# lucidrains/phenaki-pytorch

Measured on AMD Instinct MI355X. Metric: cvivit_encode_frames_per_sec, higher is better.
Workload: dtype bf16; 1 GPU; BASELINE configs[1]: C-ViViT (dim 512, patch 32, tpatch 2, depth 4+4, LFQ 65536) encode video -> token ids, (8,3,17,256,256) f32 per GPU resident in HBM; global_batch=8, parallelism=batch-shard x1, no data-path collective, hip_graph=True

## Files before the change

### include/phenaki_hip.h

```cpp
#ifndef PHENAKI_HIP_H
#define PHENAKI_HIP_H

#ifdef __cplusplus
extern "C" {
#endif

#define PK_OK 0
#define PK_EINVAL (-1)
#define PK_EALIGN (-2)
#define PK_ELAUNCH (-3)

int pk_gemm(int dtype, int a_is_f32, const void* A, int lda, const void* W, int ldw, int M, int N, int K,
            const float* bias, const float* res, int ldr, void* C, int ldc, int out_is_f32, int act,
            const int* a_rows, void* stream);

int pk_gemm_ex(int dtype, int a_is_f32, const void* A, int lda, const void* W, int ldw, int M, int N, int K,
               const float* bias, const float* res, int ldr, void* C, int ldc, int out_is_f32, int act,
               const int* a_rows, int a_nrows, int variant, void* C2, int ldc2, const float* ln_s, const float* ln_t,
               float ln_eps, const int* row_off, const int* col_off, float* stats_out, const float* ln_stats, int dup_rows,
               void* stream);
int pk_gemm_auto_variant(int dtype, int a_is_f32, int M, int N, int K, int lda, int ldw, int a_nrows);

int pk_layernorm(const float* x, int ldx, const float* gamma, const float* beta, float eps, void* out, int ldo,
                 int out_kind, float* out2, int ldo2, void* raw, int ldraw, int M, int D, int grp, int gstride,
// ... 220 lines not shown
                          const float* gscale_dev, void* stream);
int pk_ema_multi(const long long* table, int count, float weight, void* stream);
int pk_attn_train_prep(const float* q, long long ldq, const float* kv, long long ldkv, const float* null_kv, const float* q_scale, const float* k_scale,
                       float scale, float* Qh, float* Kh, float* Vh, int S, int heads, int n, int n_kv, int nnull, void* stream);
int pk_attn_train_prep_bwd(const float* q, long long ldq, const float* kv, long long ldkv, const float* null_kv, const float* q_scale, const float* k_scale,
                           float scale, const float* dQh, const float* dKh, const float* dVh, float* dq, long long lddq, float* dkv, long long lddkv,
                           float* pq, float* pk, float* dnull, int S, int heads, int n, int n_kv, int nnull, void* stream);
int pk_attn_bwd_work(int S, int heads, int n, int n_kv, int nnull);
int pk_attn_bwd_ws(const float* Qh, const float* Kh, const float* Vh, const void* O, long long ldo, int o_bf16, const float* dO, long long lddo,
                   const float* bias, const unsigned char* kmask, const float* slopes, int causal, float* dQh, float* dKh, float* dVh, float* dS,
                   float* lse, float* Drow, int S, int heads, int n, int n_kv, int nnull, int split_bf16, float* work, long long work_floats,
                   const pk_dropout* drop, void* stream);

int pk_im2col(const float* x, int B, int H, int W, int C, int kh, int kw, int stride, int pad, float* cols, long long ldc, void* stream);
int pk_col2im(const float* cols, long long ldc, int B, int H, int W, int C, int kh, int kw, int stride, int pad, float* dx, void* stream);
int pk_nchw_to_rows(const float* img, int B, int C, int H, int W, int Cp, float* rows, void* stream);
int pk_rows_to_nchw(const float* rows, int B, int C, int H, int W, int Cp, float* img, void* stream);
int pk_pick_frames(float* video, const int* frame, int B, int C, int F, int H, int W, float* img, int place, void* stream);
int pk_bmm(const float* A, long long lda, long long sA, int tA, const float* B, long long ldb, long long sB, int tB, float* C, long long ldc,
           long long sC, int batch, int M, int N, int K, int accumulate, void* stream);
int pk_row_softmax(const float* a, const float* b, const float* c, float* out, long long M, int n, int mode, void* stream);
int pk_row_l2scale(const float* x, const float* sc, const float* dz, const float* gx, const float* gsc, float* o0, float* o1, float* o2,
                   long long M, int d, int mode, void* stream);
int pk_row_ln_bwd2(const float* x, const float* gamma, const float* dy, const float* u, const float* w, float eps, float* grad_x,
                   float* grad_gamma_rows, float* grad_dy, long long M, int D, void* stream);

int pk_conv3x3(int dtype, int a_is_f32, const void* x, int B, int H, int W, int C, const void* Wm, int ldw, int Co, const float* bias, int act,
               const void* gate, int ldg, int gate_is_f32, void* y, int ldy, int out_is_f32, int tile, void* stream);
int pk_maxpool2x2(int is_f32, const void* x, int B, int H, int W, int C, void* y, void* stream);
int pk_maxpool2x2_bwd(int is_f32, const void* x, const float* dy, int B, int H, int W, int C, float* dx, void* stream);
int pk_adaptive_avgpool(int is_f32, const void* x, int B, int H, int W, int C, float* out, void* stream);
int pk_adaptive_avgpool_bwd(const float* dy, int B, int H, int W, int C, float* dx, void* stream);

int pk_frame_sqerr_parts(int H, int W);
int pk_frame_ssim_parts(int H, int W);
int pk_frame_sqerr(const float* a, const float* b, int B, int C, int F, int H, int W, float clamp_hi, float data_range, double* partials,
                   long long nparts, float* mse, float* psnr, void* stream);
int pk_frame_ssim(const float* a, const float* b, int B, int C, int F, int H, int W, float clamp_hi, float data_range, double* partials,
                  long long nparts, float* ssim, void* stream);
int pk_code_usage(const int* counts, int V, double* out, void* stream);

int pk_set_cache_policy(unsigned mask);
int pk_get_cache_policy();

int pk_gemm_epilogue_form(int dtype, int variant, int ln_kind, int vec_ok, int act, int out_is_f32, int has_bias, int has_res, int has_c2,
                          int has_stats_out, int has_scatter, int dup_rows, int pol, int pol_res);
int pk_gemm_ex_form(int dtype, int a_is_f32, const void* A, int lda, const void* W, int ldw, int M, int N, int K, const float* bias,
                    const float* res, int ldr, void* C, int ldc, int out_is_f32, int act, const int* a_rows, int a_nrows, int variant,
                    void* C2, int ldc2, const float* ln_s, const float* ln_t, float ln_eps, const int* row_off, const int* col_off,
                    float* stats_out, const float* ln_stats, int dup_rows);
int pk_set_gemm_hot_forms(int on);
int pk_get_gemm_hot_forms();

#ifdef __cplusplus
}
#endif
#endif
```

### phenaki_pytorch_amd/_lib.py

```python
import ctypes
import os

import torch

_HERE = os.path.dirname(os.path.abspath(__file__))
LIB_PATH = os.environ.get('PK_LIB_PATH') or os.path.join(_HERE, 'libphenaki_hip.so')

_P = ctypes.c_void_p
_I = ctypes.c_int
_F = ctypes.c_float
_L = ctypes.c_long
_LL = ctypes.c_longlong
_ULL = ctypes.c_ulonglong

SIGNATURES = {
    'pk_gemm': [_I, _I, _P, _I, _P, _I, _I, _I, _I, _P, _P, _I, _P, _I, _I, _I, _P, _P],
    'pk_gemm_ex': [_I, _I, _P, _I, _P, _I, _I, _I, _I, _P, _P, _I, _P, _I, _I, _I, _P, _I, _I, _P, _I, _P, _P, _F, _P, _P, _P, _P, _I, _P],
    'pk_gemm_auto_variant': [_I, _I, _I, _I, _I, _I, _I, _I],
    'pk_layernorm': [_P, _I, _P, _P, _F, _P, _I, _I, _P, _I, _P, _I, _I, _I, _I, _I, _I, _I, _I, _P],
    'pk_rmsnorm': [_P, _I, _P, _F, _P, _P, _I, _I, _I, _I, _P],
    'pk_gated_gelu_tanh': [_P, _I, _P, _I, _I, _I, _I, _P],
    'pk_l2norm_rows': [_P, _I, _P, _I, _I, _I, _I, _P],
    'pk_patchify_ln': [_P, _I, _I, _I, _I, _I, _I, _I, _I, _I, _I, _P, _P, _F, _P, _I, _I, _P],
    'pk_patch_embed': [_P, _I, _I, _I, _I, _I, _I, _I, _I, _F, _I,
# ... 76 lines not shown
    'pk_mul': [_P, _P, _P, _LL, _P],
    'pk_peg_wgrad_parts': [_LL],
    'pk_peg_bwd': [_P, _P, _P, _P, _P, _I, _I, _I, _I, _I, _I, _P],
    'pk_embed_bwd': [_P, _P, _F, _P, _P, _I, _I, _I, _P],
    'pk_bias_gather': [_P, _I, _P, _I, _P, _I, _I, _P],
    'pk_bias_scatter': [_P, _P, _I, _P, _I, _I, _I, _P],
    'pk_sum_batch': [_P, _LL, _I, _P, _LL, _P],
    'pk_sum_batch_multi': [_P, _I, _P],
    'pk_peg_adjoint': [_P, _P, _P, _I, _I, _I, _I, _I, _I, _P],
    'pk_colsum_multi': [_P, _I, _P],
    'pk_reduce_multi': [_P, _I, _P, _I, _P],
    'pk_pack_multi': [_P, _I, _P],
    'pk_pack_table_prepare': [_P, _I],
    'pk_pack_table': [_P, _I, _I, _P],
    'pk_bce_head': [_P, _LL, _P, _P, _P, _F, _P, _P, _P, _P, _LL, _P, _P, _I, _I, _P],
    'pk_attn_train_prep': [_P, _LL, _P, _LL, _P, _P, _P, _F, _P, _P, _P, _I, _I, _I, _I, _I, _P],
    'pk_attn_train_prep_bwd': [_P, _LL, _P, _LL, _P, _P, _P, _F, _P, _P, _P, _P, _LL, _P, _LL, _P, _P, _P, _I, _I, _I, _I, _I, _P],
    'pk_gemm_splitk': [_I, _P, _I, _P, _I, _I, _I, _I, _I, _P, _I, _P, _I, _P],
    'pk_adamw': [_P, _P, _P, _P, _F, _F, _F, _F, _F, _I, _LL, _P],
    'pk_adamw_multi': [_P, _I, _F, _F, _F, _F, _F, _I, _P],
    'pk_grad_sumsq_parts': [_P, _I],
    'pk_grad_sumsq': [_P, _I, _P, _LL, _P],
    'pk_grad_clip_coef': [_P, _LL, _F, _P, _P],
    'pk_scale_multi': [_P, _I, _P, _P],
    'pk_adamw_multi_scaled': [_P, _I, _F, _F, _F, _F, _F, _I, _P, _P],
    'pk_ema_multi': [_P, _I, _F, _P],
    'pk_attn_bwd_ws': [_P, _P, _P, _P, _LL, _I, _P, _LL, _P, _P, _P, _I, _P, _P, _P, _P, _P, _P, _I, _I, _I, _I, _I, _I, _P, _LL, _P, _P],
    'pk_attn_bwd_work': [_I, _I, _I, _I, _I],
    'pk_im2col': [_P, _I, _I, _I, _I, _I, _I, _I, _I, _P, _LL, _P],
    'pk_col2im': [_P, _LL, _I, _I, _I, _I, _I, _I, _I, _I, _P, _P],
    'pk_nchw_to_rows': [_P, _I, _I, _I, _I, _I, _P, _P],
    'pk_rows_to_nchw': [_P, _I, _I, _I, _I, _I, _P, _P],
    'pk_pick_frames': [_P, _P, _I, _I, _I, _I, _I, _P, _I, _P],
    'pk_bmm': [_P, _LL, _LL, _I, _P, _LL, _LL, _I, _P, _LL, _LL, _I, _I, _I, _I, _I, _P],
    'pk_row_softmax': [_P, _P, _P, _P, _LL, _I, _I, _P],
    'pk_row_l2scale': [_P, _P, _P, _P, _P, _P, _P, _P, _LL, _I, _I, _P],
    'pk_row_ln_bwd2': [_P, _P, _P, _P, _P, _F, _P, _P, _P, _LL, _I, _P],
    'pk_conv3x3': [_I, _I, _P, _I, _I, _I, _I, _P, _I, _I, _P, _I, _P, _I, _I, _P, _I, _I, _I, _P],
    'pk_maxpool2x2': [_I, _P, _I, _I, _I, _I, _P, _P],
    'pk_maxpool2x2_bwd': [_I, _P, _P, _I, _I, _I, _I, _P, _P],
    'pk_adaptive_avgpool': [_I, _P, _I, _I, _I, _I, _P, _P],
    'pk_adaptive_avgpool_bwd': [_P, _I, _I, _I, _I, _P, _P],
    'pk_frame_sqerr_parts': [_I, _I],
    'pk_frame_ssim_parts': [_I, _I],
    'pk_frame_sqerr': [_P, _P, _I, _I, _I, _I, _I, _F, _F, _P, _LL, _P, _P, _P],
    'pk_frame_ssim': [_P, _P, _I, _I, _I, _I, _I, _F, _F, _P, _LL, _P, _P],
    'pk_code_usage': [_P, _I, _P, _P],
    'pk_set_cache_policy': [ctypes.c_uint],
    'pk_get_cache_policy': [],
    'pk_gemm_epilogue_form': [_I] * 14,
    'pk_gemm_ex_form': [_I, _I, _P, _I, _P, _I, _I, _I, _I, _P, _P, _I, _P, _I, _I, _I, _P, _I, _I, _P, _I, _P, _P, _F, _P, _P, _P, _P, _I],
    'pk_set_gemm_hot_forms': [_I],
    'pk_get_gemm_hot_forms': [],
}

_ERR = {-1: 'PK_EINVAL (bad shape/size/flag)', -2: 'PK_EALIGN (pointer/stride alignment)', -3: 'PK_ELAUNCH (HIP launch failed)'}

_lib = None
_AB_OPTIONAL = ('pk_set_cache_policy', 'pk_get_cache_policy', 'pk_gemm_epilogue_form', 'pk_gemm_ex_form', 'pk_set_gemm_hot_forms', 'pk_get_gemm_hot_forms',
                'pk_vocab_ce_reg', 'pk_ce_grad_slab_reg', 'pk_vocab_weight_mean', 'pk_vocab_weight_mean_words')


def load():
    global _lib
    if _lib is None:
        if not os.path.exists(LIB_PATH):
            raise RuntimeError(f'{LIB_PATH} is missing: run `python -m phenaki_pytorch_amd.build` '
                               '(the MI355X build has no CPU / eager fallback)')
        lib = ctypes.CDLL(LIB_PATH)
        for name, args in SIGNATURES.items():
            if name in _AB_OPTIONAL and 'PK_LIB_PATH' in os.environ and not hasattr(lib, name):
                continue
            fn = getattr(lib, name)
            fn.argtypes = args
            fn.restype = _I
        _lib = lib
    return _lib


def _check(rc, name):
    if rc != 0:
        raise RuntimeError(f'{name} failed: {_ERR.get(rc, rc)}')


def ptr(t):
    return None if t is None else t.data_ptr()


def f32p(t, name='parameter', rows_ok=False):
    if t is None:
        return None
    if t.dtype != torch.float32 or not (t.is_contiguous() or (rows_ok and t.stride(-1) == 1)):
        raise RuntimeError(f'{name}: the MI355X kernels read this tensor as contiguous float32, got {t.dtype} '
                           f'{"contiguous" if t.is_contiguous() else "strided"} (keep the module in float32; the compute '
                           'precision is chosen with set_compute_dtype, not with .half()/.bfloat16())')
    return t.data_ptr()


def stream(t=None):
    if t is None:
        return torch.cuda.current_stream().cuda_stream
    idx = t.device.index
    cur = _current_device()
    if idx is not None and idx != cur:
        raise RuntimeError(f'operand on cuda:{idx} but the current device is cuda:{cur}: '
                           'call torch.cuda.set_device(...) first (one process per GPU)')
    return _raw_stream(cur)


_raw_stream = getattr(torch._C, '_cuda_getCurrentRawStream', None) or (lambda i: torch.cuda.current_stream(i).cuda_stream)
_current_device = getattr(torch._C, '_cuda_getDevice', None) or torch.cuda.current_device


def require_device(t, name='tensor'):
    if not t.is_cuda:
        raise RuntimeError(f'{name} is on {t.device}: the MI355X build runs on HIP devices only (no CPU fallback)')


F32, BF16, BF16X3 = 0, 1, 2
ACT_NONE, ACT_GEGLU, ACT_LEAKY, ACT_RELU = 0, 1, 2, 3


def tdtype(dtype):
    return torch.bfloat16 if dtype == BF16 else torch.float32


def split_planes(w32):
    n, k = w32.shape
    assert k % 32 == 0 and w32.dtype == torch.float32
    hi = w32.to(torch.bfloat16)
    lo = (w32 - hi.float()).to(torch.bfloat16)
    img = torch.cat((hi.view(n, k // 32, 32), lo.view(n, k // 32, 32)), dim=-1).contiguous()
    return img.view(n, 2 * k).view(torch.float32)



CP_PLAIN, CP_WT, CP_NT = 0, 1, 2
CP_STORE_SITES = ('gemm', 'qkv_attn', 'peg', 'ln', 'patch_wide', 'patch_finish')
CP_LOAD_SITES = ('ld_video', 'ld_partials', 'ld_residual')
CP_SITES = CP_STORE_SITES + CP_LOAD_SITES


def cache_policy_mask(**sites):
    mask = 0
    for name, pol in sites.items():
        mask |= int(pol) << (2 * CP_SITES.index(name))
    return mask


def set_cache_policy(mask):
    _check(load().pk_set_cache_policy(int(mask)), 'pk_set_cache_policy')


def get_cache_policy():
    return load().pk_get_cache_policy()


EPI_GENERIC, EPI_OUT, EPI_FF2A, EPI_FF2B, EPI_FF1 = 0, 1, 2, 3, 4


def set_gemm_hot_forms(on):
    _check(load().pk_set_gemm_hot_forms(1 if on else 0), 'pk_set_gemm_hot_forms')


def get_gemm_hot_forms():
    return load().pk_get_gemm_hot_forms()


def gemm_epilogue_form(dtype, variant, *, ln_kind=0, vec_ok=1, act=ACT_NONE, out_is_f32=1, bias=0, res=0, C2=0, stats_out=0, scatter=0,
                       dup_rows=0, pol=0, pol_res=0):
    return load().pk_gemm_epilogue_form(dtype, variant, ln_kind, int(vec_ok), act, int(out_is_f32), int(bool(bias)), int(bool(res)), int(bool(C2)),
                                        int(bool(stats_out)), int(bool(scatter)), int(dup_rows), int(pol), int(pol_res))


def _gemm_args(dtype, A, W, M, N, K, *, C, bias=None, res=None, act=ACT_NONE, a_rows=None, lda=None, ldc=None, variant=0, C2=None, ln=None,
               scatter=None, stats_out=None, ln_stats=None, dup_rows=0):
    a_is_f32 = 1 if A.dtype == torch.float32 else 0
    out_is_f32 = 1 if C.dtype == torch.float32 else 0
    lda = A.stride(-2) if lda is None else lda
    ldc = (C.stride(-2) if scatter is None else N) if ldc is None else ldc
    ldr = res.stride(-2) if res is not None else 0
    return (dtype, a_is_f32, ptr(A), lda, ptr(W), W.stride(0), M, N, K, f32p(bias, 'bias'), f32p(res, 'residual'), ldr,
            ptr(C), ldc, out_is_f32, act, ptr(a_rows), A.shape[0] if a_rows is not None else M, variant,
            ptr(C2), C2.stride(-2) if C2 is not None else 0, ptr(ln[0]) if ln else None, ptr(ln[1]) if ln else None,
            float(ln[2]) if ln else 0., ptr(scatter[0]) if scatter else None, ptr(scatter[1]) if scatter else None,
            ptr(stats_out) if stats_out is not None else None, ptr(ln_stats) if ln_stats is not None else None, int(dup_rows))


def gemm_form(dtype, A, W, M, N, K, **kw):
    rc = load().pk_gemm_ex_form(*_gemm_args(dtype, A, W, M, N, K, **kw))
    if rc < 0:
        _check(rc, 'pk_gemm_ex_form')
    return rc


def gemm(dtype, A, W, M, N, K, *, C, bias=None, res=None, act=ACT_NONE, a_rows=None, lda=None, ldc=None, variant=0, C2=None, ln=None,
         scatter=None, stats_out=None, ln_stats=None, dup_rows=0):
    rc = load().pk_gemm_ex(*_gemm_args(dtype, A, W, M, N, K, C=C, bias=bias, res=res, act=act, a_rows=a_rows, lda=lda, ldc=ldc, variant=variant, C2=C2,
                                       ln=ln, scatter=scatter, stats_out=stats_out, ln_stats=ln_stats, dup_rows=dup_rows), stream(C))
    _check(rc, 'pk_gemm_ex')
    return C


def layernorm(x, gamma, beta, M, D, *, out=None, out2=None, raw=None, eps=1e-5, remap=(0, 0, 0), perm=(0, 0), ldx=None):
    tt = out if out is not None else raw
    out_kind = 1 if (tt is not None and tt.dtype == torch.bfloat16) else 0
    rc = load().pk_layernorm(f32p(x, 'x', rows_ok=True), x.stride(-2) if ldx is None else ldx, f32p(gamma, 'LayerNorm gamma'), f32p(beta, 'LayerNorm beta'), eps,
                             ptr(out), out.stride(-2) if out is not None else 0, out_kind,
                             ptr(out2), out2.stride(-2) if out2 is not None else 0,
                             ptr(raw), raw.stride(-2) if raw is not None else 0, M, D, *remap, *perm, stream(x))
    _check(rc, 'pk_layernorm')


def patchify_ln(video, f0, nt, pt, ph, pw, weight, bias, out, eps=1e-5):
    B, C, F, H, W = video.shape
    rc = load().pk_patchify_ln(f32p(video, 'video'), B, C, F, H, W, f0, nt, pt, ph, pw, f32p(weight, 'LayerNorm weight'), f32p(bias, 'LayerNorm bias'), eps,
                               ptr(out), out.stride(0), 1 if out.dtype == torch.bfloat16 else 0, stream(video))
    _check(rc, 'pk_patchify_ln')

# ... 1008 lines not shown
```

### phenaki_pytorch_amd/build.py

```python
import os
import subprocess
import sys
from concurrent.futures import ThreadPoolExecutor

HERE = os.path.dirname(os.path.abspath(__file__))
CSRC = os.path.join(HERE, 'csrc')
OBJ = os.path.join(HERE, 'csrc', '_obj')
LIB = os.path.join(HERE, 'libphenaki_hip.so')
SOURCES = ['gemm.hip', 'qkv.hip', 'qkv_attn.hip', 'norm.hip', 'patch.hip', 'patch_embed.hip', 'elementwise.hip', 'attn.hip', 'sampler.hip', 'train.hip',
           'attn_train.hip', 'conv.hip', 'lfq_aux.hip', 'vq_train.hip', 'step_tail.hip', 'vgg.hip', 'metrics.hip']
HEADERS = ['common.hpp', 'gemm_core.hpp', 'gemm_dma.hpp', 'gemm_p8.hpp']
FLAGS = ['--offload-arch=gfx950', '-O3', '-std=c++17', '-fPIC'] + os.environ.get('PK_EXTRA_HIPCC_FLAGS', '').split()


def hipcc():
    for c in (os.environ.get('HIPCC'), '/opt/rocm/bin/hipcc', 'hipcc'):
        if c and (os.path.isabs(c) and os.path.exists(c) or not os.path.isabs(c)):
            return c
    return 'hipcc'


def _newer(target, deps):
    if not os.path.exists(target):
        return True
    t = os.path.getmtime(target)
    return any(os.path.getmtime(d) > t for d in deps)


def build(force=False, verbose=True):
    os.makedirs(OBJ, exist_ok=True)
    hdrs = [os.path.join(CSRC, h) for h in HEADERS]
    jobs = []
    for s in SOURCES:
        src = os.path.join(CSRC, s)
        obj = os.path.join(OBJ, s.replace('.hip', '.o'))
        if force or _newer(obj, [src] + hdrs):
            jobs.append((src, obj))

    def compile_one(job):
        src, obj = job
        cmd = [hipcc()] + FLAGS + ['-c', src, '-o', obj]
        r = subprocess.run(cmd, capture_output=True, text=True)
        return src, r.returncode, r.stdout + r.stderr

    if jobs:
        with ThreadPoolExecutor(max_workers=min(len(jobs), os.cpu_count() or 4)) as ex:
            for src, rc, out in ex.map(compile_one, jobs):
                if verbose:
                    print(f'[build] {os.path.basename(src)}: {"ok" if rc == 0 else "FAILED"}')
                if rc != 0:
                    raise RuntimeError(f'hipcc failed on {src}:\n{out}')
    objs = [os.path.join(OBJ, s.replace('.hip', '.o')) for s in SOURCES]
    if force or jobs or _newer(LIB, objs):
        cmd = [hipcc(), '--offload-arch=gfx950', '-shared', '-fPIC', '-o', LIB] + objs
        r = subprocess.run(cmd, capture_output=True, text=True)
        if r.returncode != 0:
            raise RuntimeError('link failed:\n' + r.stdout + r.stderr)
        if verbose:
            print(f'[build] linked {LIB}')
    return LIB


if __name__ == '__main__':
    build(force='--force' in sys.argv)
# ... 1 lines not shown
```

### phenaki_pytorch_amd/csrc/gemm.hip

```cpp
#include "gemm_dma.hpp"
#include "gemm_p8.hpp"

namespace pk {

enum { ACT_NONE = 0, ACT_GEGLU = 1, ACT_LEAKY = 2, ACT_RELU = 3 };

struct GemmEpilogue {
    const float* bias;
    const float* res;
    void* C;
    int ldr, ldc;
    int out_f32;
    int act;
    int vec_ok;
    void* C2;
    int ldc2;
    const float* ln_s; const float* ln_t; float ln_eps;
    const int* row_off; const int* col_off;
    float* stats_out; const float* ln_stats; int stats_np;
    int dup_rows;
    int pol, pol_res;
};

constexpr int STATS_CHUNK = 32;
// ... 199 lines not shown
#pragma unroll
                    for (int r = 0; r < 4; ++r) v[r] = v[r] > 0.f ? v[r] : 0.1f * v[r];
                }
                if (e.act == ACT_RELU) {
#pragma unroll
                    for (int r = 0; r < 4; ++r) v[r] = fmaxf(v[r], 0.f);
                }
                if (!LNF) v += r4[ii][j];
                else if (e.res && live) v += pol_load16(e_pol_res, e.res + (size_t)m * e.ldr + n);
                if (live) {
                    const size_t o = e.row_off ? (size_t)((long)roff[ii] + (long)coff[j]) : (size_t)m * e.ldc + n;
                    if (POLC::on && e.row_off && o >= ((size_t)1 << 30)) store4(Cf + o, v);
                    else if (e.out_f32) store4(po, Cf, o, v); else store4(po, Ct, o, v);
                    if (e.C2) store4(e_pol, C2, (size_t)m * e.ldc2 + n, v);
                    if (e.dup_rows) {
                        const size_t od = o + (size_t)e.dup_rows * e.ldc;
                        if (e.out_f32) store4(po, Cf, od, v); else store4(po, Ct, od, v);
                        if (e.C2) store4(e_pol, C2, (size_t)(m + e.dup_rows) * e.ldc2 + n, v);
                    }
                    if (TN == 2 && e.stats_out) {
#pragma unroll
                        for (int r = 0; r < 4; ++r) {
                            const float x = (sizeof(T) == 2 && (e.C2 || !e.out_f32)) ? bf2f(f2bf(v[r])) : v[r];
                            ps += x; pq += x * x;
                        }
                    }
                }
            }
            if (TN == 2 && e.stats_out) {
                ps += __shfl_xor(ps, 16); pq += __shfl_xor(pq, 16);
                ps += __shfl_xor(ps, 32); pq += __shfl_xor(pq, 32);
                const int chunk = (n0 + wn * 16 * TN) / STATS_CHUNK;
                if (g == 0 && m < M && chunk < e.stats_np)
                    store2(e_pol, e.stats_out, ((size_t)m * e.stats_np + chunk) * 2, ps, pq);
            }
        }
    }
}

template <typename T, int TM, int TN, int WN = 2, bool LNF = false, int FORM = EPI_GENERIC>
__device__ __forceinline__ void gemm_epilogue(const f32x4 (&acc)[TM][TN], int M, int N, const GemmEpilogue& e, int m0, int n0,
                                              const float* rsum = nullptr, const float* rsq = nullptr, int K = 1) {
    if constexpr (FORM != EPI_GENERIC) {
        gemm_epilogue_vec<T, TM, TN, WN, LNF, CpOff, FORM>(acc, M, N, e, m0, n0, rsum, rsq, K);
        return;
    }
    if (!e.vec_ok) {
        if (!LNF) gemm_epilogue_scalar<T, TM, TN, WN>(acc, M, N, e, m0, n0);
        return;
    }
    if (e.pol | e.pol_res) gemm_epilogue_vec<T, TM, TN, WN, LNF, CpOn>(acc, M, N, e, m0, n0, rsum, rsq, K);
    else gemm_epilogue_vec<T, TM, TN, WN, LNF, CpOff>(acc, M, N, e, m0, n0, rsum, rsq, K);
}

template <typename T, typename TA, int TM, int TN>
__global__ __launch_bounds__(256) void gemm_kernel(const GemmOperands p, const GemmEpilogue e) {
    using Tile = GemmTile<T, TA, TM, TN>;
    extern __shared__ __attribute__((aligned(16))) char smem[];
    const int m0 = blockIdx.x * Tile::BM, n0 = blockIdx.y * Tile::BN;
    f32x4 acc[TM][TN];
#pragma unroll
    for (int i = 0; i < TM; ++i)
#pragma unroll
        for (int j = 0; j < TN; ++j) acc[i][j] = f32x4{0, 0, 0, 0};
    Tile::run(p, m0, n0, smem, acc);
    gemm_epilogue<T, TM, TN>(acc, p.M, p.N, e, m0, n0);
}

template <typename Tile>
constexpr int lds_waves_per_simd() {
    const int wgs = 163840 / Tile::SMEM, w = wgs * (Tile::THREADS / 64) / 4;
    return w < 1 ? 1 : (w > 8 ? 8 : w);
}

template <typename T, int TM, int TN, int WM, int WN, int STAGES, int ROWB, int PW, int LNF = 0, int FORM = EPI_GENERIC>
__global__ __launch_bounds__(64 * (WM * WN + PW))
__attribute__((amdgpu_waves_per_eu(lds_waves_per_simd<GemmDma<T, TM, TN, WM, WN, STAGES, ROWB, PW>>(), 8)))
void gemm_dma_kernel(const GemmOperands p, const GemmEpilogue e, int a_nrows) {
    using Tile = GemmDma<T, TM, TN, WM, WN, STAGES, ROWB, PW>;
    extern __shared__ __attribute__((aligned(16))) char smem[];
    const int MT = (p.M + Tile::BM - 1) / Tile::BM, cmax = (MT + 7) / 8, NTn = (p.N + Tile::BN - 1) / Tile::BN;
    const int xcd = blockIdx.x & 7, idx = blockIdx.x >> 3;
    const int mstart = xcd * MT / 8, mcount = (xcd + 1) * MT / 8 - mstart;
    int m0, n0;
    if (p.plain_map) {
        if ((int)blockIdx.x >= MT * NTn) return;
        m0 = (blockIdx.x % MT) * Tile::BM;
        n0 = (blockIdx.x / MT) * Tile::BN;
    } else {
        int ml, ntile;
        if (!xcd_panel_tile(idx, cmax, mcount, NTn, p.panel, ml, ntile)) return;
        m0 = (mstart + ml) * Tile::BM;
        n0 = ntile * Tile::BN;
    }
    PK_TL_KERNEL(0);
    f32x4 acc[TM][TN];
#pragma unroll
    for (int i = 0; i < TM; ++i)
#pragma unroll
        for (int j = 0; j < TN; ++j) acc[i][j] = f32x4{0, 0, 0, 0};
    if constexpr (LNF == 1) {
        float rsum[TM], rsq[TM];
        if (!Tile::template run_stats<2>(p, a_nrows, m0, n0, smem, acc, rsum, rsq)) return;
        gemm_epilogue<T, TM, TN, WN, true>(acc, p.M, p.N, e, m0, n0, rsum, rsq, p.K);
    } else if constexpr (LNF == 2) {
        constexpr int TPR = Tile::THREADS / Tile::BM;
// ... 162 lines not shown
                for (int j = 0; j < 2; ++j) acc[a][b][i][j] = f32x4{0, 0, 0, 0};
    Tile::run(p, a_nrows, m0, n0, smem, acc);
    gemm_epilogue<bf16, 4, 2, 4>(acc[0][0], p.M, p.N, e, m0, n0);
    gemm_epilogue<bf16, 4, 2, 4>(acc[0][1], p.M, p.N, e, m0, n0 + 128);
    gemm_epilogue<bf16, 4, 2, 4>(acc[1][0], p.M, p.N, e, m0 + 128, n0);
    gemm_epilogue<bf16, 4, 2, 4>(acc[1][1], p.M, p.N, e, m0 + 128, n0 + 128);
}

static int launch_p8_splitk(const GemmOperands& p, const GemmEpilogue& e, int a_nrows, int splits, long ba, long bw, long bc, hipStream_t s) {
    using Tile = GemmP8;
    static LdsOptIn lds;
    if (lds.raise(reinterpret_cast<const void*>(&gemm_p8_splitk_kernel), Tile::SMEM) != PK_OK) return PK_ELAUNCH;
    const int MT = (p.M + Tile::BM - 1) / Tile::BM, NT = (p.N + Tile::BN - 1) / Tile::BN;
    hipLaunchKernelGGL(gemm_p8_splitk_kernel, dim3(MT * NT, splits), dim3(Tile::THREADS), Tile::SMEM, s, p, e, a_nrows, ba, bw, bc);
    PK_CHECK_LAUNCH();
    return PK_OK;
}

}

using namespace pk;

static inline bool al16(const void* p) { return (reinterpret_cast<uintptr_t>(p) & 15) == 0; }

static bool dma_possible(int dtype, int a_is_f32, int N, int K, int lda, int ldw, int a_nrows) {
    const int bk = dtype == 1 ? 64 : 32;
    const int kpad = (K + bk - 1) / bk * bk;
    const size_t el = dtype == 1 ? 2 : 4;
    return !(dtype == 1 && a_is_f32) && ldw >= kpad &&
           (size_t)a_nrows * lda * el < 0xFFFFFFF0ull && (size_t)N * ldw * el < 0xFFFFFFF0ull;
}

static int auto_variant(int dtype, int a_is_f32, int M, int N, int K, int lda, int ldw, int a_nrows) {
    const long blocks128 = (long)((M + 127) / 128) * ((N + 127) / 128);
    if (!dma_possible(dtype, a_is_f32, N, K, lda, ldw, a_nrows)) return blocks128 >= 384 ? 2 : 1;
    static const long t128 = getenv("PK_GEMM_T128") ? atol(getenv("PK_GEMM_T128")) : 256;
    if (dtype != 0 && blocks128 >= t128 && blocks128 < 384 && K <= 1024) return 27;
    if (dtype == 1 && K >= 2048 && (long)((M + 255) / 256) * ((N + 255) / 256) >= 512) return 50;
    if (blocks128 >= t128) return dtype == 2 ? 9 : 24;
    if (K >= 2048) return dtype == 1 ? 33 : 3;
    return 8;
}

extern "C" int pk_gemm_auto_variant(int dtype, int a_is_f32, int M, int N, int K, int lda, int ldw, int a_nrows) {
    return auto_variant(dtype, a_is_f32, M, N, K, lda, ldw, a_nrows);
}

static int& hot_forms_word() {
    static int on = [] { const char* e_ = getenv("PK_GEMM_HOT_FORMS"); return e_ ? (atoi(e_) != 0 ? 1 : 0) : 1; }();
    return on;
}
extern "C" int pk_set_gemm_hot_forms(int on) { hot_forms_word() = on ? 1 : 0; return PK_OK; }
extern "C" int pk_get_gemm_hot_forms() { return hot_forms_word(); }

extern "C" int pk_gemm_epilogue_form(int dtype, int variant, int ln_kind, int vec_ok, int act, int out_is_f32, int has_bias, int has_res,
                                     int has_c2, int has_stats_out, int has_scatter, int dup_rows, int pol, int pol_res) {
    if (dtype != 1 || !vec_ok || pol || pol_res || has_bias || has_scatter || dup_rows) return EPI_GENERIC;
    if (variant == 8 && ln_kind == 0 && act == ACT_NONE && out_is_f32 && has_res) {
        if (has_stats_out) return has_c2 ? EPI_OUT : EPI_GENERIC;
        return has_c2 ? EPI_FF2A : EPI_FF2B;
    }
    if (variant == 24 && ln_kind == 2 && act == ACT_GEGLU && !out_is_f32 && !has_res && !has_c2 && !has_stats_out) return EPI_FF1;
    return EPI_GENERIC;
}

static int gemm_ex(int dtype, int a_is_f32, const void* A, int lda, const void* W, int ldw,
                   int M, int N, int K, const float* bias, const float* res, int ldr,
                   void* C, int ldc, int out_is_f32, int act, const int* a_rows, int a_nrows,
                   int variant, void* C2, int ldc2, const float* ln_s, const float* ln_t, float ln_eps,
                   const int* row_off, const int* col_off, float* stats_out, const float* ln_stats, int dup_rows, void* stream, int* form_only) {
    if (M <= 0 || N <= 0 || K <= 0 || !A || !W || !C) return PK_EINVAL;
    if (dtype != 0 && dtype != 1 && dtype != 2) return PK_EINVAL;
    if (act < 0 || act > 3) return PK_EINVAL;
    const int eps_w = dtype == 1 ? 8 : 4;
    const int eps_a = (dtype == 1 && !a_is_f32) ? 8 : 4;
    if (K % eps_w || ldw % eps_w || lda % eps_a) return PK_EALIGN;
    if (dtype == 1 && a_is_f32 && (K % 8)) return PK_EALIGN;
    if (!al16(A) || !al16(W)) return PK_EALIGN;
    if (dtype != 1 && !a_is_f32) return PK_EINVAL;
    if (dtype == 2 && C2) return PK_EINVAL;
    if (act == ACT_GEGLU && (N & 1)) return PK_EINVAL;
    if (act == ACT_GEGLU && res) return PK_EINVAL;
    if (a_rows && a_nrows <= 0) return PK_EINVAL;
    if (!a_rows) a_nrows = M;
    GemmOperands p{A, W, a_rows, lda, ldw, M, N, K, 0, N >= 8192 ? krot_default() : 0};
    GemmEpilogue e{bias, res, C, ldr, ldc, out_is_f32, act, 0, C2, ldc2, ln_s, ln_t, ln_eps, row_off, col_off, stats_out, ln_stats,
                   ((ln_stats ? K : N) + STATS_CHUNK - 1) / STATS_CHUNK, dup_rows};
    bool v = (N % 4 == 0) && (ldc % 4 == 0) && al16(C) && (!bias || al16(bias)) && (!res || (al16(res) && ldr % 4 == 0));
    if (act == ACT_GEGLU) v = v && (ldc % 2 == 0) && ((reinterpret_cast<uintptr_t>(C) & 7) == 0);
    e.vec_ok = v ? 1 : 0;
    e.pol = cache_policy_for(CPS_GEMM, row_off ? 0 : ((size_t)(M - 1 + dup_rows) * ldc + N) * (size_t)(out_is_f32 || dtype != 1 ? 4 : 2));
    e.pol_res = cache_policy(CPS_LD_RES);
    if (C2 && (!v || !out_is_f32 || act == ACT_GEGLU || dtype != 1 || (ldc2 & 3) || (reinterpret_cast<uintptr_t>(C2) & 7))) return PK_EINVAL;
    if ((ln_s == nullptr) != (ln_t == nullptr)) return PK_EINVAL;
    if ((row_off == nullptr) != (col_off == nullptr)) return PK_EINVAL;
    if (row_off && (!v || !out_is_f32 || act == ACT_GEGLU || res || C2)) return PK_EINVAL;
    if (ln_stats && (!ln_s || stats_out || (reinterpret_cast<uintptr_t>(ln_stats) & 7))) return PK_EINVAL;
    if (stats_out && (!v || act == ACT_GEGLU || row_off || (reinterpret_cast<uintptr_t>(stats_out) & 7))) return PK_EINVAL;
    if (dup_rows < 0 || (dup_rows && (!v || act == ACT_GEGLU || row_off || stats_out || dup_rows < M))) return PK_EINVAL;
    hipStream_t s = reinterpret_cast<hipStream_t>(stream);

    const bool dma_ok = dma_possible(dtype, a_is_f32, N, K, lda, ldw, a_nrows);
    if (variant >= 100) { p.plain_map = 1; variant -= 100; }
    if (variant == 0) variant = auto_variant(dtype, a_is_f32, M, N, K, lda, ldw, a_nrows);
    if (variant >= 3 && !dma_ok) return PK_EINVAL;
    const int form = !hot_forms_word() ? EPI_GENERIC
                   : pk_gemm_epilogue_form(dtype, variant, ln_s ? (ln_stats ? 2 : 1) : 0, e.vec_ok, act, out_is_f32, bias != nullptr, res != nullptr,
                                           C2 != nullptr, stats_out != nullptr, row_off != nullptr, dup_rows, e.pol, e.pol_res);
    if (ln_s) {
        if (!dma_ok || !v || !al16(ln_s) || !al16(ln_t) || a_rows) return PK_EINVAL;
        if (form_only) { *form_only = form; return PK_OK; }
        if (form == EPI_FF1) return launch_dma<bf16, 4, 2, 2, 2, 4, 128, 0, 2, EPI_FF1>(p, e, a_nrows, s);
        const bool big = variant == 24 || variant == 2 || variant == 9 || variant == 50;
        if (ln_stats) {
            if (dtype == 1) return big ? launch_dma<bf16, 4, 2, 2, 2, 4, 128, 0, 2>(p, e, a_nrows, s) : launch_dma<bf16, 2, 2, 2, 2, 2, 128, 0, 2>(p, e, a_nrows, s);
            if (dtype == 2) return big ? launch_dma<bf16x3, 4, 4, 2, 2, 2, 128, 0, 2>(p, e, a_nrows, s) : launch_dma<bf16x3, 2, 2, 2, 2, 2, 128, 0, 2>(p, e, a_nrows, s);
            return big ? launch_dma<float, 4, 2, 2, 2, 4, 128, 0, 2>(p, e, a_nrows, s) : launch_dma<float, 2, 2, 2, 2, 2, 128, 0, 2>(p, e, a_nrows, s);
        }
        if (dtype == 1) return big ? launch_dma<bf16, 4, 2, 2, 2, 4, 128, 0, 1>(p, e, a_nrows, s) : launch_dma<bf16, 2, 2, 2, 2, 2, 128, 0, 1>(p, e, a_nrows, s);
        if (dtype == 2) return big ? launch_dma<bf16x3, 4, 4, 2, 2, 2, 128, 0, 1>(p, e, a_nrows, s) : launch_dma<bf16x3, 2, 2, 2, 2, 2, 128, 0, 1>(p, e, a_nrows, s);
        return big ? launch_dma<float, 4, 2, 2, 2, 4, 128, 0, 1>(p, e, a_nrows, s) : launch_dma<float, 2, 2, 2, 2, 2, 128, 0, 1>(p, e, a_nrows, s);
    }
    if (stats_out && !(dma_ok && (variant == 8 || variant == 24 || variant == 27 || variant == 33 || variant == 50 || (variant == 3 && dtype != 1)))) return PK_EINVAL;
    if (form_only) { *form_only = form; return PK_OK; }
    if (form == EPI_OUT) return launch_dma<bf16, 2, 2, 2, 2, 2, 128, 0, 0, EPI_OUT>(p, e, a_nrows, s);
    if (form == EPI_FF2A) return launch_dma<bf16, 2, 2, 2, 2, 2, 128, 0, 0, EPI_FF2A>(p, e, a_nrows, s);
    if (form == EPI_FF2B) return launch_dma<bf16, 2, 2, 2, 2, 2, 128, 0, 0, EPI_FF2B>(p, e, a_nrows, s);
    if (dtype == 1) {
        switch (variant) {
            case 1: return a_is_f32 ? launch_v1<bf16, float, 2, 2>(p, e, s) : launch_v1<bf16, bf16, 2, 2>(p, e, s);
            case 2: return a_is_f32 ? launch_v1<bf16, float, 4, 4>(p, e, s) : launch_v1<bf16, bf16, 4, 4>(p, e, s);
            case 8: return launch_dma<bf16, 2, 2, 2>(p, e, a_nrows, s);
            case 9: return launch_dma<bf16, 4, 4, 2>(p, e, a_nrows, s);
            case 24: return launch_dma<bf16, 4, 2, 2, 2, 4>(p, e, a_nrows, s);
            case 33: return launch_dma<bf16, 2, 2, 3, 2, 2, 128, 2>(p, e, a_nrows, s);
            case 27: return launch_dma<bf16, 4, 2, 2, 2, 2>(p, e, a_nrows, s);
            case 50: return launch_p8(p, e, a_nrows, s);
            default: return PK_EINVAL;
        }
    }
    if (dtype == 2) {
        if (!dma_ok) return PK_EINVAL;
        switch (variant) {
            case 3: return launch_dma<bf16x3, 2, 2, 4>(p, e, a_nrows, s);
            case 8: return launch_dma<bf16x3, 2, 2, 2>(p, e, a_nrows, s);
            case 9: return launch_dma<bf16x3, 4, 4, 2>(p, e, a_nrows, s);
            case 24: return launch_dma<bf16x3, 4, 2, 2, 2, 4>(p, e, a_nrows, s);
            case 27: return launch_dma<bf16x3, 4, 2, 2, 2, 2>(p, e, a_nrows, s);
            default: return PK_EINVAL;
        }
    }
    switch (variant) {
        case 1: return launch_v1<float, float, 2, 2>(p, e, s);
        case 2: return launch_v1<float, float, 4, 4>(p, e, s);
        case 3: return launch_dma<float, 2, 2, 4>(p, e, a_nrows, s);
        case 8: return launch_dma<float, 2, 2, 2>(p, e, a_nrows, s);
        case 9: return launch_dma<float, 4, 4, 2>(p, e, a_nrows, s);
        case 24: return launch_dma<float, 4, 2, 2, 2, 4>(p, e, a_nrows, s);
        default: return PK_EINVAL;
    }
}

extern "C" int pk_gemm_ex(int dtype, int a_is_f32, const void* A, int lda, const void* W, int ldw,
                          int M, int N, int K, const float* bias, const float* res, int ldr,
// ... 65 lines not shown
```

Measured before the change: 178,800 frames/s.

## Add LDS-resident A-panel kernel for LN-fused GEGLU FF1 GEMM

Adds a specialised FF1 GEMM kernel for K=1024. It loads a 128-row A panel into LDS once per block, then streams W tiles through registers across a split of N among several workers per panel. The epilogue of each step (LayerNorm fold, GEGLU, bf16 store) runs during the next step's MMA to overlap store and compute. It is on by default only for M of 4608 or 9216, which are the workload shapes, and the worker count comes from the CU count divided by the number of panels. This trades a general tiled kernel for a specialised one with heavy LDS use (128 KB) and hand-built pipelining.

```diff
diff --git a/include/phenaki_hip.h b/include/phenaki_hip.h
--- a/include/phenaki_hip.h
+++ b/include/phenaki_hip.h
@@ -296,6 +296,11 @@
 int pk_set_gemm_hot_forms(int on);
 int pk_get_gemm_hot_forms();
 
+int pk_set_ff1_resident(int mode);
+int pk_get_ff1_resident();
+int pk_set_ff1_resident_workers(int n);
+int pk_get_ff1_resident_launches();
+
 #ifdef __cplusplus
 }
 #endif
diff --git a/phenaki_pytorch_amd/_lib.py b/phenaki_pytorch_amd/_lib.py
--- a/phenaki_pytorch_amd/_lib.py
+++ b/phenaki_pytorch_amd/_lib.py
@@ -152,13 +152,18 @@
     'pk_gemm_ex_form': [_I, _I, _P, _I, _P, _I, _I, _I, _I, _P, _P, _I, _P, _I, _I, _I, _P, _I, _I, _P, _I, _P, _P, _F, _P, _P, _P, _P, _I],
     'pk_set_gemm_hot_forms': [_I],
     'pk_get_gemm_hot_forms': [],
+    'pk_set_ff1_resident': [_I],
+    'pk_get_ff1_resident': [],
+    'pk_set_ff1_resident_workers': [_I],
+    'pk_get_ff1_resident_launches': [],
 }
 
 _ERR = {-1: 'PK_EINVAL (bad shape/size/flag)', -2: 'PK_EALIGN (pointer/stride alignment)', -3: 'PK_ELAUNCH (HIP launch failed)'}
 
 _lib = None
 _AB_OPTIONAL = ('pk_set_cache_policy', 'pk_get_cache_policy', 'pk_gemm_epilogue_form', 'pk_gemm_ex_form', 'pk_set_gemm_hot_forms', 'pk_get_gemm_hot_forms',
-                'pk_vocab_ce_reg', 'pk_ce_grad_slab_reg', 'pk_vocab_weight_mean', 'pk_vocab_weight_mean_words')
+                'pk_vocab_ce_reg', 'pk_ce_grad_slab_reg', 'pk_vocab_weight_mean', 'pk_vocab_weight_mean_words',
+                'pk_set_ff1_resident', 'pk_get_ff1_resident', 'pk_set_ff1_resident_workers', 'pk_get_ff1_resident_launches')
 
 
 def load():
@@ -265,6 +270,22 @@
 
 def get_gemm_hot_forms():
     return load().pk_get_gemm_hot_forms()
+
+
+def set_ff1_resident(mode):
+    _check(load().pk_set_ff1_resident(int(mode)), 'pk_set_ff1_resident')
+
+
+def get_ff1_resident():
+    return load().pk_get_ff1_resident()
+
+
+def set_ff1_resident_workers(n):
+    _check(load().pk_set_ff1_resident_workers(int(n)), 'pk_set_ff1_resident_workers')
+
+
+def ff1_resident_launches():
+    return load().pk_get_ff1_resident_launches()
 
 
 def gemm_epilogue_form(dtype, variant, *, ln_kind=0, vec_ok=1, act=ACT_NONE, out_is_f32=1, bias=0, res=0, C2=0, stats_out=0, scatter=0,
diff --git a/phenaki_pytorch_amd/build.py b/phenaki_pytorch_amd/build.py
--- a/phenaki_pytorch_amd/build.py
+++ b/phenaki_pytorch_amd/build.py
@@ -9,7 +9,7 @@
 LIB = os.path.join(HERE, 'libphenaki_hip.so')
 SOURCES = ['gemm.hip', 'qkv.hip', 'qkv_attn.hip', 'norm.hip', 'patch.hip', 'patch_embed.hip', 'elementwise.hip', 'attn.hip', 'sampler.hip', 'train.hip',
            'attn_train.hip', 'conv.hip', 'lfq_aux.hip', 'vq_train.hip', 'step_tail.hip', 'vgg.hip', 'metrics.hip']
-HEADERS = ['common.hpp', 'gemm_core.hpp', 'gemm_dma.hpp', 'gemm_p8.hpp']
+HEADERS = ['common.hpp', 'gemm_core.hpp', 'gemm_dma.hpp', 'gemm_p8.hpp', 'gemm_resident.hpp']
 FLAGS = ['--offload-arch=gfx950', '-O3', '-std=c++17', '-fPIC'] + os.environ.get('PK_EXTRA_HIPCC_FLAGS', '').split()
 
 
diff --git a/phenaki_pytorch_amd/csrc/gemm.hip b/phenaki_pytorch_amd/csrc/gemm.hip
--- a/phenaki_pytorch_amd/csrc/gemm.hip
+++ b/phenaki_pytorch_amd/csrc/gemm.hip
@@ -275,6 +275,10 @@
     if (e.pol | e.pol_res) gemm_epilogue_vec<T, TM, TN, WN, LNF, CpOn>(acc, M, N, e, m0, n0, rsum, rsq, K);
     else gemm_epilogue_vec<T, TM, TN, WN, LNF, CpOff>(acc, M, N, e, m0, n0, rsum, rsq, K);
 }
+
+}
+#include "gemm_resident.hpp"
+namespace pk {
 
 template <typename T, typename TA, int TM, int TN>
 __global__ __launch_bounds__(256) void gemm_kernel(const GemmOperands p, const GemmEpilogue e) {
@@ -543,6 +547,54 @@
 }
 extern "C" int pk_set_gemm_hot_forms(int on) { hot_forms_word() = on ? 1 : 0; return PK_OK; }
 extern "C" int pk_get_gemm_hot_forms() { return hot_forms_word(); }
+
+static int& ff1_resident_word() {
+    static int v = [] { const char* e_ = getenv("PK_FF1_RESIDENT"); const int x = e_ ? atoi(e_) : 1; return x < 0 || x > 2 ? 1 : x; }();
+    return v;
+}
+static int& ff1_resident_workers_word() {
+    static int v = [] { const char* e_ = getenv("PK_FF1_RESIDENT_WORKERS"); const int x = e_ ? atoi(e_) : 0; return x > 0 ? x : 0; }();
+    return v;
+}
+static int& ff1_resident_launch_count() { static int n = 0; return n; }
+extern "C" int pk_set_ff1_resident(int mode) { if (mode < 0 || mode > 2) return PK_EINVAL; ff1_resident_word() = mode; return PK_OK; }
+extern "C" int pk_get_ff1_resident() { return ff1_resident_word(); }
+extern "C" int pk_set_ff1_resident_workers(int n) { if (n < 0 || n > 4096) return PK_EINVAL; ff1_resident_workers_word() = n; return PK_OK; }
+extern "C" int pk_get_ff1_resident_launches() { return ff1_resident_launch_count(); }
+
+static bool ff1_resident_window(int M) { return M == 4608 || M == 9216; }
+
+static int gemm_n_cu() {
+    static int cus[64] = {};
+    int dev = 0;
+    if (hipGetDevice(&dev) != hipSuccess || dev < 0 || dev >= 64) return 256;
+    if (!cus[dev]) {
+        int n = 0;
+        if (hipDeviceGetAttribute(&n, hipDeviceAttributeMultiprocessorCount, dev) != hipSuccess || n <= 0) n = 256;
+        cus[dev] = n;
+    }
+    return cus[dev];
+}
+
+static int ff1_resident_workers(int form, int requested, int M, int K) {
+    if (form != EPI_FF1 || K != 64 * FR_NT || !ff1_resident_word()) return 0;
+    const int forced = ff1_resident_workers_word();
+    if (forced) return forced;
+    if (requested != 0) return 0;
+    if (ff1_resident_word() == 1 && !ff1_resident_window(M)) return 0;
+    const int w = gemm_n_cu() / ((M + 127) / 128);
+    return w < 1 ? 1 : w;
+}
+
+static int launch_ff1_resident(const GemmOperands& p, const GemmEpilogue& e, int workers, hipStream_t s) {
+    static LdsOptIn lds;
+    if (lds.raise(reinterpret_cast<const void*>(&ff1_resident_kernel), FR_SMEM) != PK_OK) return PK_ELAUNCH;
+    const long units = (long)((p.M + 127) / 128) * workers;
+    hipLaunchKernelGGL(ff1_resident_kernel, dim3((unsigned)(8 * ((units + 7) / 8))), dim3(512), FR_SMEM, s, p, e, workers);
+    PK_CHECK_LAUNCH();
+    ff1_resident_launch_count() = (ff1_resident_launch_count() + 1) & 0x7fffffff;
+    return PK_OK;
+}
 
 extern "C" int pk_gemm_epilogue_form(int dtype, int variant, int ln_kind, int vec_ok, int act, int out_is_f32, int has_bias, int has_res,
                                      int has_c2, int has_stats_out, int has_scatter, int dup_rows, int pol, int pol_res) {
@@ -592,6 +644,7 @@
     hipStream_t s = reinterpret_cast<hipStream_t>(stream);
 
     const bool dma_ok = dma_possible(dtype, a_is_f32, N, K, lda, ldw, a_nrows);
+    const int requested = variant;
     if (variant >= 100) { p.plain_map = 1; variant -= 100; }
     if (variant == 0) variant = auto_variant(dtype, a_is_f32, M, N, K, lda, ldw, a_nrows);
     if (variant >= 3 && !dma_ok) return PK_EINVAL;
@@ -601,6 +654,7 @@
     if (ln_s) {
         if (!dma_ok || !v || !al16(ln_s) || !al16(ln_t) || a_rows) return PK_EINVAL;
         if (form_only) { *form_only = form; return PK_OK; }
+        if (const int rw = ff1_resident_workers(form, requested, M, K)) return launch_ff1_resident(p, e, rw, s);
         if (form == EPI_FF1) return launch_dma<bf16, 4, 2, 2, 2, 4, 128, 0, 2, EPI_FF1>(p, e, a_nrows, s);
         const bool big = variant == 24 || variant == 2 || variant == 9 || variant == 50;
         if (ln_stats) {
diff --git a/phenaki_pytorch_amd/csrc/gemm_resident.hpp b/phenaki_pytorch_amd/csrc/gemm_resident.hpp
--- /dev/null
+++ b/phenaki_pytorch_amd/csrc/gemm_resident.hpp
@@ -0,0 +1,193 @@
+#pragma once
+
+namespace pk {
+
+constexpr int FR_NT = 8;
+constexpr int FR_PANEL = FR_NT * 128 * 128;
+constexpr int FR_SMEM = FR_PANEL + 128 * 8;
+
+__device__ __forceinline__ void fr_wait_block(int kt) {
+    switch (kt) {
+        case 0: wait_vmcnt<14>(); break; case 1: wait_vmcnt<12>(); break; case 2: wait_vmcnt<10>(); break; case 3: wait_vmcnt<8>(); break;
+        case 4: wait_vmcnt<6>(); break; case 5: wait_vmcnt<4>(); break; case 6: wait_vmcnt<2>(); break; default: wait_vmcnt<0>(); break;
+    }
+}
+
+struct FrNoEpi { __device__ __forceinline__ void operator()(int) const {} };
+template <int NF, bool FIRST, int NFP = 0, typename PrevEpi = FrNoEpi>
+__device__ __forceinline__ void fr_step(const char* smem, __amdgpu_buffer_rsrc_t rsW, u32x4 (&wreg)[FR_NT][2], uint32_t nbase, int frag0, int lr, int g,
+                                        f32x4 (&acc)[NF], const PrevEpi& prev_epi = PrevEpi{}) {
+    static_assert(!(FIRST && NFP), "the first step has no step before it");
+#pragma unroll
+    for (int i = 0; i < NF; ++i) acc[i] = f32x4{0, 0, 0, 0};
+    Frag<bf16> fa[2][NF];
+    if (FIRST) {
+        fr_wait_block(0);
+        __builtin_amdgcn_s_barrier();
+    }
+#pragma unroll
+    for (int i = 0; i < NF; ++i) lds_frag(fa[0][i], smem, (frag0 + i) * 16 + lr, 0, g);
+#pragma unroll
+    for (int t = 0; t < 2 * FR_NT; ++t) {
+        const int kt = t >> 1, ch = t & 1;
+        if (t + 1 < 2 * FR_NT) {
+            const int kt1 = (t + 1) >> 1, ch1 = (t + 1) & 1;
+            if (FIRST && ch1 == 0) {
+                fr_wait_block(kt1);
+                __builtin_amdgcn_s_barrier();
+            }
+#pragma unroll
+            for (int i = 0; i < NF; ++i) lds_frag(fa[(t + 1) & 1][i], smem + kt1 * 16384, (frag0 + i) * 16 + lr, ch1, g);
+        }
+        Frag<bf16> fw;
+        fw.v = wreg[kt][ch];
+#pragma unroll
+        for (int i = 0; i < NF; ++i) acc[i] = mma(fw, fa[t & 1][i], acc[i]);
+        wreg[kt][ch] = __builtin_amdgcn_raw_buffer_load_b128(rsW, nbase + ch * 64, kt * 128, 0);
+        if (NFP == 8 && ch == 0) prev_epi(kt);
+        if (NFP == 1 && t == 0) prev_epi(0);
+        __builtin_amdgcn_sched_barrier(0);
+    }
+}
+
+__device__ __forceinline__ void fr_epi_frag(const f32x4& a, const GemmOperands& p, const GemmEpilogue& e, const float2* ls, int m0, int frag, int n,
+                                            const f32x4& s4, const f32x4& t4, int lr) {
+    bf16* __restrict__ Ct = reinterpret_cast<bf16*>(e.C);
+    const f32x4 b4 = f32x4{0, 0, 0, 0};
+    const float inv_k = 1.0f / (float)p.K;
+    const int ml = frag * 16 + lr, m = m0 + ml;
+    const float2 pr = ls[ml];
+    const bool edge = m0 + 128 > p.M || (n & ~127) + 128 > p.N;
+    const float mean = pr.x * inv_k;
+    const float var = edge ? __builtin_fmaf(inv_k, pr.y, -(mean * mean)) : __builtin_fmaf(-mean, mean, pr.y * inv_k);
+    const float rstd = __builtin_amdgcn_rsqf(fmaxf(var, 0.f) + e.ln_eps);
+    f32x4 v;
+#pragma unroll
+    for (int r = 0; r < 4; ++r) v[r] = __builtin_fmaf(rstd, __builtin_fmaf(-mean, s4[r], a[r]), t4[r]);
+    v += b4;
+    const float o0 = gelu_for<bf16>(v[1]) * v[0], o1 = gelu_for<bf16>(v[3]) * v[2];
+    if (m < p.M && n < p.N) store2(Ct + ((size_t)m * e.ldc + (n >> 1)), o0, o1);
+}
+template <int NF>
+__device__ __forceinline__ void fr_epilogue(const f32x4 (&acc)[NF], const GemmOperands& p, const GemmEpilogue& e, const float2* ls, int m0, int frag0,
+                                            int n, const f32x4& s4, const f32x4& t4, int lr) {
+#pragma unroll
+    for (int i = 0; i < NF; ++i) fr_epi_frag(acc[i], p, e, ls, m0, frag0 + i, n, s4, t4, lr);
+}
+
+__global__ __launch_bounds__(512) void ff1_resident_kernel(const GemmOperands p, const GemmEpilogue e, int workers) {
+    extern __shared__ __attribute__((aligned(16))) char smem[];
+    typedef __attribute__((address_space(3))) void* lds_ptr;
+    const int tid = threadIdx.x, lane = tid & 63;
+    const int wave = __builtin_amdgcn_readfirstlane(tid >> 6);
+    const int g = lane >> 4, lr = lane & 15;
+    const int N = p.N;
+    const int panels = (p.M + 127) / 128, units = panels * workers;
+    const int xcd = blockIdx.x & 7, idx = blockIdx.x >> 3;
+    const int u0 = (int)((long)xcd * units / 8), u1 = (int)((long)(xcd + 1) * units / 8);
+    if (idx >= u1 - u0) return;
+    const int unit = u0 + idx, panel = unit / workers, wk = unit - panel * workers;
+    const int S = (N + 15) / 16;
+    const int sb0 = (int)((long)wk * S / workers), Sw = (int)((long)(wk + 1) * S / workers) - sb0;
+    if (Sw == 0) return;
+    const int full = Sw >> 3, steps = full + (Sw & 7);
+    const int m0 = panel * 128;
+
+    const uint32_t bytesA = (uint32_t)p.M * (uint32_t)p.lda * 2u, bytesW = (uint32_t)N * (uint32_t)p.ldw * 2u;
+    __amdgpu_buffer_rsrc_t rsA = __builtin_amdgcn_make_buffer_rsrc(const_cast<void*>(p.A), 0, bytesA, 0x00020000);
+    __amdgpu_buffer_rsrc_t rsW = __builtin_amdgcn_make_buffer_rsrc(const_cast<void*>(p.W), 0, bytesW, 0x00020000);
+    auto sb_of = [&](int t) { return t < full ? sb0 + t * 8 + wave : sb0 + full * 8 + (t - full); };
+    auto w_base = [&](int t) -> uint32_t {
+        const int row = sb_of(t) * 16 + lr;
+        return (t < steps && row < N) ? (uint32_t)row * (uint32_t)p.ldw * 2u + g * 16 : bytesW;
+    };
+    auto fold_vec = [&](const float* v, int t) {
+        const int n = sb_of(t < steps ? t : 0) * 16 + g * 4;
+        return *reinterpret_cast<const f32x4*>(v + (n < N - 4 ? n : N - 4));
+    };
+
+    const int srow = tid >> 2, sq4 = tid & 3;
+    const float2* st = reinterpret_cast<const float2*>(e.ln_stats) + (size_t)min(m0 + srow, p.M - 1) * e.stats_np + sq4 * 4;
+    float2 pre[4];
+#pragma unroll
+    for (int u = 0; u < 4; ++u) pre[u] = st[u];
+    f32x4 s4 = fold_vec(e.ln_s, 0), t4 = fold_vec(e.ln_t, 0);
+    u32x4 wreg[FR_NT][2];
+    {
+        const uint32_t base = w_base(0);
+#pragma unroll
+        for (int kt = 0; kt < FR_NT; ++kt)
+#pragma unroll
+            for (int ch = 0; ch < 2; ++ch) wreg[kt][ch] = __builtin_amdgcn_raw_buffer_load_b128(rsW, base + ch * 64, kt * 128, 0);
+    }
+    __builtin_amdgcn_sched_barrier(0);
+    {
+        const int lrow = lane >> 3, lslot = lane & 7, srcslot = lslot ^ lrow;
+#pragma unroll
+        for (int kt = 0; kt < FR_NT; ++kt)
+#pragma unroll
+            for (int j = 0; j < 2; ++j) {
+                const int piece = wave * 2 + j;
+                const int gm = m0 + piece * 8 + lrow;
+                const uint32_t off = gm < p.M ? (uint32_t)gm * (uint32_t)p.lda * 2u + srcslot * 16 : bytesA;
+                __builtin_amdgcn_raw_ptr_buffer_load_lds(rsA, (lds_ptr)(smem + kt * 16384 + piece * 1024), 16, off, kt * 128, 0, 0);
+            }
+    }
+    __builtin_amdgcn_sched_barrier(0);
+    float2* ls = reinterpret_cast<float2*>(smem + FR_PANEL);
+    {
+        float su = 0.f, sq = 0.f;
+#pragma unroll
+        for (int u = 0; u < 4; ++u) { su += pre[u].x; sq += pre[u].y; }
+        su += __shfl_xor(su, 1); sq += __shfl_xor(sq, 1);
+        su += __shfl_xor(su, 2); sq += __shfl_xor(sq, 2);
+        const uint32_t ls_off = (uint32_t)(uintptr_t)(lds_ptr)(ls + srow);
+        const uint64_t pair = ((uint64_t)__builtin_bit_cast(uint32_t, sq) << 32) | __builtin_bit_cast(uint32_t, su);
+        if (sq4 == 0) asm volatile("ds_write_b64 %0, %1" ::"v"(ls_off), "v"(pair) : "memory");
+        asm volatile("s_waitcnt lgkmcnt(0)" ::: "memory");
+    }
+
+    auto n_of = [&](int t) { return sb_of(t) * 16 + g * 4; };
+    int np = n_of(0);
+    f32x4 s4p = s4, t4p = t4;
+    f32x4 prev1[1];
+    int t = 1;
+    bool owed1 = true;
+    if (full > 0) {
+        f32x4 prev[8];
+        fr_step<8, true>(smem, rsW, wreg, w_base(1), 0, lr, g, prev);
+#pragma unroll 1
+        for (; t < full; ++t) {
+            const f32x4 s4c = fold_vec(e.ln_s, t), t4c = fold_vec(e.ln_t, t);
+            f32x4 acc[8];
+            fr_step<8, false, 8>(smem, rsW, wreg, w_base(t + 1), 0, lr, g, acc, [&](int i) { fr_epi_frag(prev[i], p, e, ls, m0, i, np, s4p, t4p, lr); });
+#pragma unroll
+            for (int i = 0; i < 8; ++i) prev[i] = acc[i];
+            np = n_of(t); s4p = s4c; t4p = t4c;
+        }
+        if (t < steps) {
+            const f32x4 s4c = fold_vec(e.ln_s, t), t4c = fold_vec(e.ln_t, t);
+            fr_step<1, false, 8>(smem, rsW, wreg, w_base(t + 1), wave, lr, g, prev1, [&](int i) { fr_epi_frag(prev[i], p, e, ls, m0, i, np, s4p, t4p, lr); });
+            np = n_of(t); s4p = s4c; t4p = t4c;
+            ++t;
+        } else {
+            fr_epilogue<8>(prev, p, e, ls, m0, 0, np, s4p, t4p, lr);
+            owed1 = false;
+        }
+    } else {
+        fr_step<1, true>(smem, rsW, wreg, w_base(1), wave, lr, g, prev1);
+    }
+    if (owed1) {
+#pragma unroll 1
+        for (; t < steps; ++t) {
+            const f32x4 s4c = fold_vec(e.ln_s, t), t4c = fold_vec(e.ln_t, t);
+            f32x4 acc[1];
+            fr_step<1, false, 1>(smem, rsW, wreg, w_base(t + 1), wave, lr, g, acc, [&](int) { fr_epi_frag(prev1[0], p, e, ls, m0, wave, np, s4p, t4p, lr); });
+            prev1[0] = acc[0];
+            np = n_of(t); s4p = s4c; t4p = t4c;
+        }
+        fr_epi_frag(prev1[0], p, e, ls, m0, wave, np, s4p, t4p, lr);
+    }
+}
+
+}
```

New measurement: 184,000 frames/s (median of 6 runs). +2.9%, better.
